# modelscope/dash-infer

Hardware: NVIDIA H100
Metric: decode tokens/sec/GPU Qwen2-7B int4-IQ b=1..64; HBM GB/s vs roofline (higher is better)
Workload: dtype bf16 activations x int4 weights (fp32 accumulate), none KV

## Files before the change

dash-infer_b200/csrc/wq_gemm.cu:

```cuda
#include <cstdio>
#include <cstdlib>
#include <cstring>
#include <map>
#include <mutex>
#include <new>

#include "b2_common.cuh"
#include "comm_shared.cuh"
#include "wq_gemm_shared.cuh"

namespace b2 {

constexpr int kWarps = 8;
constexpr int kThreads = kWarps * 32 + 32;
constexpr int kStageBytes = 8192;
static_assert(kBN == kWarps * 16, "one n16 tile per consumer warp");

struct GemmParams {
  const uint8_t* packed;
  const float2* sz;
  const __nv_bfloat16* A;
  int64_t lda;
  __nv_bfloat16* C;
  int64_t ldc;
  const __nv_bfloat16* bias;
  const __nv_bfloat16* residual;
  float* ws;
  unsigned* counters;
  int M, N, K, Np, KT, NG, S;
  int group_tiles;
  int quanta;
  int xt;
  int nst_log2;
  int act;
  float alpha;
  int cluster;
  int norm_self;
  const __nv_bfloat16* norm_gamma;
  float norm_inv_hidden, norm_eps;
  int comm_on;
  CommDev comm;
};

template <int WBITS>
struct WTraits {
  static constexpr int TILE_BYTES = Image<WBITS>::kTileBytes;
  static constexpr int TPS = kStageBytes / TILE_BYTES > 0 ? kStageBytes / TILE_BYTES : 1;
  static constexpr int STAGE_BYTES = TPS * TILE_BYTES;
};

__device__ __forceinline__ void named_bar_sync(int id, int n) { asm volatile("bar.sync %0, %1;" ::"r"(id), "r"(n) : "memory"); }

// ... 598 lines not shown
          v = (n & 1) ? (b >> 4) : (b & 0xF);
        } else if (WBITS == 8) {
          v = static_cast<const uint8_t*>(src)[(int64_t)k * N + n];
        } else {
          v = static_cast<const uint16_t*>(src)[(int64_t)k * N + n];
        }
      }
      word |= (v ^ flip) << (WBITS * ((e >> 1) + (e & 1) * I::kKPerWord / 2));
    }
    dst[i] = I::kRotated ? (word << 3) | (word >> 29) : word;
  }
}

__global__ void pack_sz_kernel(float2* __restrict__ dst, const __nv_bfloat16* __restrict__ scales,
                               const __nv_bfloat16* __restrict__ zeros, const __nv_bfloat16* __restrict__ scales2,
                               const __nv_bfloat16* __restrict__ zeros2, int pair, int G, int N, int Np, float zbias, int fp16) {
  const int64_t total = (int64_t)G * Np;
  for (int64_t i = blockIdx.x * (int64_t)blockDim.x + threadIdx.x; i < total; i += (int64_t)gridDim.x * blockDim.x) {
    const int np = i % Np, gi = i / Np;
    const int r = np & (kBN - 1), ng = np / kBN;
    const int n = pair ? ng * 64 + (r & 63) : np;
    const __nv_bfloat16* sc = (pair && r >= 64) ? scales2 : scales;
    const __nv_bfloat16* zr = (pair && r >= 64) ? zeros2 : zeros;
    float2 v = make_float2(0.f, 0.f);
    if (n < N) {
      const __nv_bfloat16 sv = sc[(int64_t)gi * N + n], zv = zr[(int64_t)gi * N + n];
      v = fp16 ? make_float2(Ft<true>::to_f(sv), Ft<true>::to_f(zv) + zbias) : make_float2(Ft<false>::to_f(sv), Ft<false>::to_f(zv) + zbias);
    }
    dst[i] = v;
  }
}

}

using namespace b2;

struct Plan {
  bool valid = false;
  int S = 1, xt = 1, smem = 0, quanta = 1, nst_log2 = 2;
  bool cluster = false;
};

struct b2_gemm_wq {
  b2_gemm_wq_desc d;
  int Kp = 0, Np = 0, KT = 0, NG = 0, G = 1, group_tiles = 0;
  int group_k = 0;
  size_t packed_bytes = 0;
  void* packed = nullptr;
  bool own_packed = false;
  float2* sz = nullptr;
  bool own_sz = false;
  unsigned* counters = nullptr;
  Plan plans[2];
  int tc_S = 0;
  bool pair = false;
  int device = 0;
};

typedef void (*gemm_kernel_t)(const GemmParams);

static gemm_kernel_t pick_kernel(int wbits, bool grouped, int mt, bool fp16) {
  return with_wbits(wbits, [&](auto W) {
    return with_flag(grouped, [&](auto G) {
      return with_flag(mt == 1, [&](auto MT1) {
        return with_flag(fp16, [&](auto H) { return wq_gemm_kernel<W, MT1 ? 1 : 2, G && W != 16, H>; });
      });
    });
  });
}
static int stage_bytes_of(int wbits) { return with_wbits(wbits, [](auto W) { return WTraits<W>::STAGE_BYTES; }); }

cudaError_t b2::raise_smem_limit(const void* kern, int smem) {
  static std::mutex mu;
  static std::map<const void*, int> limit;
  std::lock_guard<std::mutex> lk(mu);
  int& cur = limit[kern];
  if (smem <= cur) return cudaSuccess;
  cudaError_t e = cudaFuncSetAttribute(kern, cudaFuncAttributeMaxDynamicSharedMemorySize, smem);
  if (e == cudaSuccess) cur = smem;
  return e;
}

static int make_plan(b2_gemm_wq* h, int mti) {
  Plan& pl = h->plans[mti];
  if (pl.valid) return B2_OK;
  const int mt = 1 << mti, MP = 8 * mt;
  const bool grouped = h->group_tiles > 0;
  const int gt = grouped ? h->group_tiles : 1;
  const int quanta = h->KT / gt;
  const int sms = sm_count();
  gemm_kernel_t kern = pick_kernel(h->d.wbits, grouped, mt, h->d.ft == B2_DT_F16);
  const int ring_kb = env_int("B2_GEMM_RING_KB", 32);
  auto log2_stages = [&](int kb) {
    int l = 1;
    while ((2 << l) * stage_bytes_of(h->d.wbits) <= kb * 1024) ++l;
    return l;
  };
  int nst_log2 = log2_stages(ring_kb);
  const int tps = with_wbits(h->d.wbits, [](auto W) { return WTraits<W>::TPS; });
  const int xq = gt > tps ? gt : tps;
  const int x_budget = env_int("B2_GEMM_XBYTES", 20 * 1024);
  int xt_cap = (x_budget / (MP + 1) - 16) / 128;
  xt_cap = xt_cap / xq * xq;
  if (xt_cap < xq) xt_cap = xq;
  auto smem_for = [&](int xt, int nl2) {
    const int gpc = grouped ? xt / gt : 1;
    return (1 << nl2) * stage_bytes_of(h->d.wbits) + (MP + 1) * (xt * 128 + 16) + MP * kBN * 4 + MP * gpc * 4 + 2 * MP * 4 + 16 + 8 +
// ... 141 lines not shown
  if (int st = launch_failed("pack_weights")) return st;
  if (d.wbits != 16) {
    if (!h->sz || !h->own_sz) {
      B2_CUDA_TRY(cudaMalloc(&h->sz, sizeof(float2) * (size_t)h->G * h->Np));
      h->own_sz = true;
    }
    const float b0 = d.ft == B2_DT_F16 ? 128.f : 16.f;
    const float zbias = d.wbits == 4 ? b0 : (d.qtype == B2_DT_I8 ? 17.f * b0 + 128.f : 17.f * b0);
    const int64_t tot = (int64_t)h->G * h->Np;
    pack_sz_kernel<<<(int)((tot + 255) / 256), 256, 0, stream>>>(h->sz, (const __nv_bfloat16*)scales, (const __nv_bfloat16*)zeros,
                                                                 (const __nv_bfloat16*)scales2, (const __nv_bfloat16*)zeros2, pair,
                                                                 h->G, d.N, h->Np, zbias, d.ft == B2_DT_F16 ? 1 : 0);
    if (int st = launch_failed("pack_sz")) return st;
  }
  return B2_OK;
}

int b2_gemm_wq_prepare_weights(b2_gemm_wq_t h, const void* qdata, const void* scales, const void* zeros,
                               void* packed_dst, void* stream_) {
  if (h && h->pair) return B2_ERR_PARAM;
  return prepare_impl(h, qdata, scales, zeros, nullptr, nullptr, nullptr, packed_dst, stream_);
}

int b2_gemm_wq_prepare_swiglu(b2_gemm_wq_t h, const void* q_gate, const void* s_gate, const void* z_gate, const void* q_up,
                              const void* s_up, const void* z_up, void* stream_) {
  if (!h || !h->pair) return B2_ERR_PARAM;
  return prepare_impl(h, q_gate, s_gate, z_gate, q_up, s_up, z_up, nullptr, stream_);
}

int b2_gemm_wq_attach_packed(b2_gemm_wq_t h, const void* packed, const void* scales_f32, const void* zeros_f32) {
  (void)zeros_f32;
  if (!h || !packed) return B2_ERR_PARAM;
  if (h->own_packed && h->packed) cudaFree(h->packed);
  h->packed = const_cast<void*>(packed);
  h->own_packed = false;
  if (scales_f32) {
    if (h->own_sz && h->sz) cudaFree(h->sz);
    h->sz = (float2*)const_cast<void*>(scales_f32);
    h->own_sz = false;
  }
  return B2_OK;
}

static int mt_index_for(int M) { return M <= 8 ? 0 : 1; }

constexpr int kTcMinM = 17;

static bool use_tc(const b2_gemm_wq* h, int M) {
  if (h->group_k > 0) return true;
  return M >= kTcMinM && (h->group_tiles == 0 || h->d.wbits == 4);
}

static void make_tc_plan(b2_gemm_wq* h) {
  if (h->tc_S > 0) return;
  const int ctas = env_int("B2_GEMM_TC_CTAS_PER_SM", 1);
  auto split_for = [&](int slots, int smax) {
    int S = slots / h->NG;
    if (S > h->KT / 4) S = h->KT / 4;
    if (S > smax) S = smax;
    return S < 1 ? 1 : S;
  };
  h->tc_S = split_for(ctas * sm_count(), env_int("B2_GEMM_TC_MAX_SPLIT", 6));
}

static size_t tc_workspace_bytes(b2_gemm_wq* h) {
  make_tc_plan(h);
  return h->tc_S <= 1 ? 16 : (size_t)h->NG * h->tc_S * kTcMaxM * kBN * sizeof(float) + 16;
}

static int run_tc(b2_gemm_wq* h, TcParams p, int M, cudaStream_t stream) {
  make_tc_plan(h);
  if (h->tc_S > 1 && !p.ws) return B2_ERR_PARAM;
  p.packed = (const uint8_t*)h->packed; p.sz = h->sz; p.counters = h->counters;
  p.N = h->d.N; p.K = h->d.K; p.Np = h->Np; p.KT = h->KT; p.NG = h->NG; p.S = h->tc_S;
  const int64_t a_row = p.a_scale ? p.lda : 2 * p.lda;
  for (int m0 = 0; m0 < M; m0 += kTcMaxM) {
    TcParams q = p;
    q.M = (M - m0) > kTcMaxM ? kTcMaxM : (M - m0);
    q.A = reinterpret_cast<const __nv_bfloat16*>(reinterpret_cast<const uint8_t*>(p.A) + m0 * a_row);
    q.C = p.C + (int64_t)m0 * p.ldc;
    if (p.residual) q.residual = p.residual + (int64_t)m0 * p.ldc;
    if (p.a_scale) {
      q.a_scale = p.a_scale + m0;
      q.tile_sums = p.tile_sums + (size_t)m0 * p.KT;
    }
    if (p.norm_sumsq) q.norm_sumsq = p.norm_sumsq + m0;
    if (p.xg_out) {
      q.sumsq_out = p.sumsq_out + m0;
      q.xg_out = p.xg_out + (int64_t)m0 * p.ldxg;
    }
    cudaError_t e = tc_launch(h->d.wbits, h->d.ft == B2_DT_F16, q, stream);
    if (e != cudaSuccess) {
      set_last_error(p.a_scale ? "wq_gemm_tc (fp8) launch" : "wq_gemm_tc launch", e);
      return B2_ERR_CUDA;
    }
  }
  return B2_OK;
}

size_t b2_gemm_wq_workspace_bytes(b2_gemm_wq_t h, int M) {
  if (!h || M <= 0) return 0;
  if (use_tc(h, M)) return tc_workspace_bytes(h);
  const int mc = M > kGemvMaxM ? kGemvMaxM : M;
  const int mti = mt_index_for(mc);
  if (make_plan(h, mti) != B2_OK) return 0;
  const Plan& pl = h->plans[mti];
  if (pl.S <= 1 || pl.cluster) return 16;
  return (size_t)h->NG * pl.S * (8 << mti) * (kBN + 1) * sizeof(float) + 16;
}

size_t b2_gemm_wq_algo_bytes(b2_gemm_wq_t h, int M) {
  if (!h) return 0;
  const b2_gemm_wq_desc& d = h->d;
  const size_t mul = h->pair ? 2 : 1;
  size_t w = mul * (size_t)d.K * d.N * d.wbits / 8;
  size_t prm = d.wbits == 16 ? 0 : mul * (size_t)2 * 2 * h->G * d.N;
  return w + prm + (size_t)2 * M * ((size_t)d.K + d.N);
}

int b2_gemm_wq_sumsq_parts(b2_gemm_wq_t h) { return h ? h->NG : 0; }

int b2_gemm_wq_run(b2_gemm_wq_t h, const void* A, int64_t lda, void* C, int64_t ldc, int M, const void* bias,
                   const void* residual, int activation, float alpha, void* workspace, size_t workspace_bytes,
                   void* stream_) {
  return b2_gemm_wq_run_fused(h, A, lda, C, ldc, M, bias, residual, activation, alpha, workspace, workspace_bytes, nullptr, stream_);
}

// ... 172 lines not shown
```

dash-infer_b200/csrc/wq_gemm_shared.cuh:

```cuda
#pragma once
#include <cuda.h>

#include <type_traits>

#include "b2_common.cuh"

namespace b2 {

constexpr int kBN = 128;
constexpr int kBK = 64;
constexpr uint32_t kMask4 = 0x00780078u;
constexpr uint32_t kMagic = 0x41804180u;
constexpr uint32_t kMagicHi = 0x43804380u;

template <int WBITS>
struct Image {
  static constexpr int kChunks = WBITS == 4 ? 2 : (WBITS == 8 ? 4 : 8);
  static constexpr int kKPerChunk = kBK / kChunks;
  static constexpr int kKPerWord = kKPerChunk / 4;
  static constexpr int kChunkBytes = kBN * 16;
  static constexpr int kTileBytes = kChunks * kChunkBytes;
  static constexpr int kTileWords = kTileBytes / 4;
  static constexpr bool kRotated = WBITS != 16;
  __host__ __device__ __forceinline__ static int swz(int c) {
    return WBITS == 4 ? 4 * (c & 1) : (WBITS == 8 ? 2 * (c & 3) : 2 * ((c >> 1) & 3));
  }
  __host__ __device__ __forceinline__ static int row_offset(int row, int c) { return (row ^ swz(c)) << 4; }
  __host__ __device__ __forceinline__ static int chunk_offset(const int& row, int c) { return c * kChunkBytes + ((row ^ swz(c)) << 4); }
};

template <typename F>
inline auto with_wbits(int wbits, F&& f) {
  if (wbits == 4) return f(std::integral_constant<int, 4>{});
  if (wbits == 8) return f(std::integral_constant<int, 8>{});
  return f(std::integral_constant<int, 16>{});
}

struct TcParams {
  const uint8_t* packed;
  const float2* sz;
  const __nv_bfloat16* A;
  int64_t lda;
  __nv_bfloat16* C;
  int64_t ldc;
  const __nv_bfloat16* bias;
  const __nv_bfloat16* residual;
  float* ws;
  unsigned* counters;
  int M, N, K, Np, KT, NG, S;
  int act;
  float alpha;
  const float* a_scale = nullptr;
  const float* tile_sums = nullptr;
  const float* norm_sumsq = nullptr;
  int norm_parts = 0, norm_ld = 0;
  float norm_inv_hidden = 0.f, norm_eps = 0.f;
  float* sumsq_out = nullptr;
  __nv_bfloat16* xg_out = nullptr;
  const __nv_bfloat16* gamma_out = nullptr;
  int64_t ldxg = 0;
  int nm;
  int group_tiles = 0;
  int group_k = 0, ngroups = 1;
};

struct Gemv2Params {
  const uint8_t* packed;
  const __nv_bfloat16* A;
  int64_t lda;
  __nv_bfloat16* C;
  int64_t ldc;
  const __nv_bfloat16* bias;
  const __nv_bfloat16* residual;
  int M, N, K, KT, NG;
  int cb_log2;
  int xt;
  int nst_log2;
  int pair;
  int act;
  float alpha;
};
struct Gemv2Plan {
  int mt, grid, smem;
};
bool gemv2_plan(Gemv2Params& p, Gemv2Plan* plan);
cudaError_t gemv2_launch(const Gemv2Params& p, const Gemv2Plan& plan, cudaStream_t stream);

constexpr int kGemvMaxM = 16;
constexpr int kTcMaxM = 64;
cudaError_t tc_launch(int wbits, bool fp16, TcParams p, cudaStream_t stream);

cudaError_t raise_smem_limit(const void* kern, int smem);

typedef CUresult (*EncodeTiledFn)(CUtensorMap*, CUtensorMapDataType, cuuint32_t, void*, const cuuint64_t*, const cuuint64_t*,
                                  const cuuint32_t*, const cuuint32_t*, CUtensorMapInterleave, CUtensorMapSwizzle,
                                  CUtensorMapL2promotion, CUtensorMapFloatOOBfill);
EncodeTiledFn encode_tiled();

}
```

dash-infer_b200/csrc/wq_gemm_tc.cu:

```cuda
#include <type_traits>

#include "b2_common.cuh"
#include "wq_gemm_shared.cuh"

namespace b2 {

constexpr int kTcThreads = 384;
constexpr int kTcNM = 64;
constexpr int kTcNSW = 6;
constexpr int kTcNSX = 3;
constexpr int kTcXTile = kTcNM * 128;

__device__ __forceinline__ void wg_fence() { asm volatile("wgmma.fence.sync.aligned;" ::: "memory"); }
__device__ __forceinline__ void wg_commit() { asm volatile("wgmma.commit_group.sync.aligned;" ::: "memory"); }
template <int N>
__device__ __forceinline__ void wg_wait() { asm volatile("wgmma.wait_group.sync.aligned %0;" ::"n"(N) : "memory"); }
__device__ __forceinline__ void wg_fence_acc(float (&d)[32]) {
#pragma unroll
  for (int i = 0; i < 32; ++i) asm volatile("" : "+f"(d[i])::"memory");
}
__device__ __forceinline__ uint64_t wg_desc(uint32_t saddr) {
  return (uint64_t)((saddr >> 4) & 0x3FFF) | ((uint64_t)1 << 16) | ((uint64_t)(1024 >> 4) << 32) | ((uint64_t)1 << 62);
}

// ... 39 lines not shown
}

__device__ __forceinline__ uint32_t tc_prmt(uint32_t a, uint32_t b, uint32_t sel) {
  uint32_t d;
  asm("prmt.b32 %0, %1, %2, %3;" : "=r"(d) : "r"(a), "r"(b), "r"(sel));
  return d;
}
__device__ __forceinline__ uint32_t lds32(uint32_t addr) {
  uint32_t v;
  asm volatile("ld.shared.u32 %0, [%1];" : "=r"(v) : "r"(addr));
  return v;
}
__device__ __forceinline__ uint32_t nib4_to_e4m3(uint32_t w_rot3, uint32_t qsh, uint32_t msel) {
  const uint32_t word = __funnelshift_r(w_rot3, w_rot3, 3);
  const uint32_t sel = (word & 0x77777777u) >> qsh;
  const uint32_t T0 = 0x44403800u, T1 = 0x4E4C4A48u, H0 = 0x53525150u, H1 = 0x57565554u;
  const uint32_t lo = tc_prmt(T0, T1, sel), hi = tc_prmt(H0, H1, sel);
  const uint32_t m = tc_prmt(word << 4, word, msel);
  uint32_t r;
  asm("lop3.b32 %0, %1, %2, %3, 0xD8;" : "=r"(r) : "r"(lo), "r"(hi), "r"(m));
  return r;
}

template <int WBITS, bool MULTI, bool A8 = false, bool GROUPED = false, bool H = false>
__global__ void __launch_bounds__(kTcThreads, 1) wq_gemm_tc_kernel(const TcParams p, const __grid_constant__ CUtensorMap amap) {
  using I = Image<WBITS>;
  constexpr int TILE_BYTES = I::kTileBytes;
  constexpr int NSW = WBITS == 16 ? 4 : kTcNSW;
  constexpr int TPS = WBITS == 4 ? 4 : 2;
  constexpr int KIND = A8 ? 2 : (H ? 1 : 0);
  static_assert(!A8 || WBITS == 4, "fp8 activations: int4 weights only");
  static_assert(!H || !A8, "fp8 activations come with bf16 outputs");
  using F = Ft<H>;
  static_assert(!GROUPED || (!A8 && WBITS != 16), "sub-channel weights: bf16 activations, int4 / int8");
  const int XTILE_LD = p.nm * 128;
  constexpr int XTPS = A8 ? TPS / 2 : TPS;
  constexpr int WSTAGE = TPS * TILE_BYTES;
  constexpr int XSTAGE = XTPS * kTcXTile;
  extern __shared__ uint8_t smem_raw[];
  uint8_t* smem = reinterpret_cast<uint8_t*>((reinterpret_cast<uintptr_t>(smem_raw) + 1023) & ~uintptr_t(1023));
  uint8_t* xring = smem;
  uint8_t* wring = xring + kTcNSX * XSTAGE;
  float* suma = reinterpret_cast<float*>(wring + NSW * WSTAGE);
  uint64_t* bars = reinterpret_cast<uint64_t*>(suma + kTcNM);
  uint64_t* wfull = bars;
  uint64_t* wfree = wfull + kTcNSW;
  uint64_t* afull = wfree + kTcNSW;
  uint64_t* xsum = afull + kTcNSX;
  uint64_t* xfree = xsum + kTcNSX;
  float* ascale = reinterpret_cast<float*>(bars) + 64;
  __shared__ int s_is_last;

  const int tid = threadIdx.x, warp = tid >> 5, lane = tid & 31;
  const int nunits = p.NG * p.S;

  if (tid == 0) {
    for (int i = 0; i < NSW; ++i) { mbar_init(&wfull[i], 1); mbar_init(&wfree[i], 8); }
    for (int i = 0; i < kTcNSX; ++i) { mbar_init(&afull[i], 1); mbar_init(&xsum[i], 2); mbar_init(&xfree[i], 8); }
    fence_mbar_init();
  }
  __syncthreads();
  pdl_launch_dependents();

  int w_pre = 0;
  const int my_units = !MULTI ? 1 : ((int)blockIdx.x < nunits) ? (nunits - (int)blockIdx.x + (int)gridDim.x - 1) / (int)gridDim.x : 0;
  auto body = [&](auto n32) {
  constexpr bool N32 = decltype(n32)::value;
  for (int uit = 0; uit < my_units; ++uit) {
  const int unit = (int)blockIdx.x + uit * (int)gridDim.x;
  const int ng = unit / p.S;
  const int s = unit - ng * p.S;
  const int kt0 = (int)((int64_t)s * p.KT / p.S), kt1 = (int)((int64_t)(s + 1) * p.KT / p.S);
  const int nt = kt1 - kt0;
  const int nst = (nt + TPS - 1) / TPS;
  const int gbase = MULTI ? uit * nst : 0;
  if (warp == 8) {
    if (lane == 0) {
      auto issue = [&](int g, const uint8_t* src, uint32_t bytes) {
        const int slot = g % NSW;
        if (g >= NSW) mbar_wait_backoff(&wfree[slot], ((g / NSW) & 1) ^ 1);
        mbar_arrive_expect_tx(&wfull[slot], bytes);
        bulk_g2s(wring + slot * WSTAGE, src, bytes, &wfull[slot]);
      };
      const uint8_t* wsrc = p.packed + ((size_t)ng * p.KT + kt0) * TILE_BYTES;
      for (int st = w_pre; st < nst; ++st) issue(gbase + st, wsrc + (size_t)st * WSTAGE, min(TPS, nt - st * TPS) * TILE_BYTES);
      w_pre = 0;
      const int nu = unit + gridDim.x;
      if (MULTI && nu < nunits) {
        const int ng2 = nu / p.S, s2 = nu - ng2 * p.S;
        const int k0 = (int)((int64_t)s2 * p.KT / p.S), k1 = (int)((int64_t)(s2 + 1) * p.KT / p.S);
        const int nt2 = k1 - k0, nst2 = (nt2 + TPS - 1) / TPS;
        const uint8_t* wsrc2 = p.packed + ((size_t)ng2 * p.KT + k0) * TILE_BYTES;
        w_pre = min(NSW, nst2);
        for (int st = 0; st < w_pre; ++st)
          issue(gbase + nst + st, wsrc2 + (size_t)st * WSTAGE, min(TPS, nt2 - st * TPS) * TILE_BYTES);
      }
    }
  } else if (warp == 9) {
    if (lane == 0) {
      pdl_wait();
      for (int st = 0; st < nst; ++st) {
        const int g = gbase + st;
        const int slot = g % kTcNSX;
        if (g >= kTcNSX) {
          const uint32_t par = ((g / kTcNSX) & 1) ^ 1;
          mbar_wait_backoff(&xfree[slot], par);
          mbar_wait_backoff(&xsum[slot], par);
        }
        const int wtiles = min(TPS, nt - st * TPS);
        const int tiles = A8 ? (wtiles + 1) / 2 : wtiles;
        mbar_arrive_expect_tx(&afull[slot], tiles * XTILE_LD);
        for (int ti = 0; ti < tiles; ++ti)
          asm volatile("cp.async.bulk.tensor.2d.shared::cluster.global.mbarrier::complete_tx::bytes [%0], [%1, {%2, %3}], [%4];"
                       ::"r"(smem_u32(xring + slot * XSTAGE + ti * kTcXTile)), "l"(reinterpret_cast<uint64_t>(&amap)),
                         "r"((kt0 + st * TPS + (A8 ? 2 * ti : ti)) * kBK), "r"(0), "r"(smem_u32(&afull[slot]))
                       : "memory");
      }
    }
  } else if (warp >= 10) {
    const int xt = tid - 320;
    float r0 = 0.f, r1 = 0.f, r2 = 0.f, r3 = 0.f;
    if (A8) {
      pdl_wait();
      if (xt < p.M) {
        const float* ts = p.tile_sums + (size_t)xt * p.KT;
        for (int kt = kt0; kt < kt1; ++kt) r0 += ts[kt];
        ascale[xt] = p.a_scale[xt];
      } else {
        ascale[xt] = 0.f;
      }
    }
    if (!A8 && p.norm_sumsq) {
      pdl_wait();
      float ss = 0.f;
      if (xt < p.M)
        for (int i = 0; i < p.norm_parts; ++i) ss += __ldcg(p.norm_sumsq + (size_t)i * p.norm_ld + xt);
      ascale[xt] = rsqrtf(ss * p.norm_inv_hidden + p.norm_eps);
    }
    for (int st = 0; st < nst; ++st) {
      const int g = gbase + st;
      const int slot = g % kTcNSX;
      mbar_wait(&afull[slot], (g / kTcNSX) & 1);
      const int tiles = (WBITS == 16 || A8 || GROUPED || xt >= p.nm) ? 0 : min(TPS, nt - st * TPS);
      for (int ti = 0; ti < tiles; ++ti) {
        const uint32_t rbase = smem_u32(xring + slot * XSTAGE + ti * kTcXTile) + xt * 128;
#pragma unroll
        for (int c = 0; c < 8; c += 2) {
          const uint4 v = lds128(rbase + ((c ^ (xt & 7)) << 4));
          const uint4 w = lds128(rbase + (((c + 1) ^ (xt & 7)) << 4));
          r0 += (F::lo(v.x) + F::hi(v.x)) + (F::lo(v.y) + F::hi(v.y));
          r1 += (F::lo(v.z) + F::hi(v.z)) + (F::lo(v.w) + F::hi(v.w));
          r2 += (F::lo(w.x) + F::hi(w.x)) + (F::lo(w.y) + F::hi(w.y));
          r3 += (F::lo(w.z) + F::hi(w.z)) + (F::lo(w.w) + F::hi(w.w));
        }
      }
      __syncwarp();
      if (lane == 0) mbar_arrive(&xsum[slot]);
    }
    suma[xt] = (r0 + r1) + (r2 + r3);
    asm volatile("bar.sync 3, 320;" ::: "memory");
  } else {
    const int wg = warp >> 2, g8 = lane >> 2, t4 = lane & 3;
    const int rr0 = wg * 64 + (warp & 3) * 16 + g8, rr1 = rr0 + 8;
    const float2 sz0 = (WBITS == 16 || GROUPED) ? make_float2(1.f, 0.f) : p.sz[ng * kBN + rr0];
    const float2 sz1 = (WBITS == 16 || GROUPED) ? make_float2(1.f, 0.f) : p.sz[ng * kBN + rr1];
    const uint32_t wring_u = smem_u32(wring), xring_u = smem_u32(xring);
    uint32_t off0[I::kChunks], off1[I::kChunks];
#pragma unroll
    for (int c = 0; c < I::kChunks; ++c) {
      off0[c] = I::chunk_offset(rr0, c);
      off1[c] = I::chunk_offset(rr1, c);
    }
    const uint32_t sh4 = 4 * t4, sh8 = 8 * (t4 & 1), qsh = 16 * (t4 & 1), msel = (t4 & 1) ? 0xFBEAu : 0xD9C8u;
    const int wa = t4 >> 1;
    auto word = [](const uint4& v, int j) { return j == 0 ? v.x : (j == 1 ? v.y : (j == 2 ? v.z : v.w)); };

    float d[32], dt[32];
#pragma unroll
    for (int i = 0; i < 32; ++i) d[i] = dt[i] = 0.f;
    int prev_xs = -1;
    for (int st = 0; st < nst; ++st) {
      const int g = gbase + st;
      const int slot = g % NSW, xs = g % kTcNSX;
      uint32_t gs2[TPS][2], gc2[TPS][2];
      if (GROUPED && p.group_k == 0) {
#pragma unroll
        for (int ti = 0; ti < TPS; ++ti) {
          const int kt = min(kt0 + st * TPS + ti, kt1 - 1);
          const float2 z0 = __ldg(p.sz + (size_t)(kt / p.group_tiles) * p.Np + ng * kBN + rr0);
          const float2 z1 = __ldg(p.sz + (size_t)(kt / p.group_tiles) * p.Np + ng * kBN + rr1);
          const float c0 = (F::kBias + 8.f - z0.y) * z0.x, c1 = (F::kBias + 8.f - z1.y) * z1.x;
          gs2[ti][0] = F::pack(z0.x, z0.x); gs2[ti][1] = F::pack(z1.x, z1.x);
          gc2[ti][0] = F::pack(c0, c0); gc2[ti][1] = F::pack(c1, c1);
        }
      }
      mbar_wait(&wfull[slot], (g / NSW) & 1);
      mbar_wait(&afull[xs], (g / kTcNSX) & 1);
      const int tiles = min(TPS, nt - st * TPS);
#pragma unroll
      for (int ti = 0; ti < TPS; ++ti) {
        if (ti < tiles) {
          const uint32_t wt = wring_u + slot * WSTAGE + ti * TILE_BYTES;
          if (A8) {
            const uint64_t bd = wg_desc(xring_u + xs * XSTAGE + (ti >> 1) * kTcXTile) + (uint64_t)(4 * (ti & 1));
            uint32_t a[2][4];
#pragma unroll
            for (int c = 0; c < 2; ++c) {
              const uint4 v0 = lds128(wt + off0[c]), v1 = lds128(wt + off1[c]);
              a[c][0] = nib4_to_e4m3(word(v0, wa), qsh, msel);
              a[c][1] = nib4_to_e4m3(word(v1, wa), qsh, msel);
              a[c][2] = nib4_to_e4m3(word(v0, 2 + wa), qsh, msel);
              a[c][3] = nib4_to_e4m3(word(v1, 2 + wa), qsh, msel);
            }
            wg_fence();
#pragma unroll
            for (int c = 0; c < 2; ++c) wg_mma<KIND, N32>(dt, a[c], bd + (uint64_t)(2 * c));
          } else {
            const uint64_t bd = wg_desc(xring_u + xs * XSTAGE + ti * kTcXTile);
            if (WBITS == 4) {
              uint32_t a[4][4];
#pragma unroll
              for (int c = 0; c < 2; ++c) {
                const uint4 v0 = lds128(wt + off0[c]), v1 = lds128(wt + off1[c]);
#pragma unroll
                for (int h = 0; h < 2; ++h) {
                  uint32_t* f = a[2 * c + h];
                  f[0] = lop3_and_or(__funnelshift_r(word(v0, 2 * h), word(v0, 2 * h), sh4), kMask4, F::kMagic);
                  f[1] = lop3_and_or(__funnelshift_r(word(v1, 2 * h), word(v1, 2 * h), sh4), kMask4, F::kMagic);
                  f[2] = lop3_and_or(__funnelshift_r(word(v0, 2 * h + 1), word(v0, 2 * h + 1), sh4), kMask4, F::kMagic);
                  f[3] = lop3_and_or(__funnelshift_r(word(v1, 2 * h + 1), word(v1, 2 * h + 1), sh4), kMask4, F::kMagic);
                  if (GROUPED) {
                    uint32_t sw[4], cw[4];
// ... 35 lines not shown
                a[kk][1] = lds32(wt + off1[2 * kk] + 4 * t4);
                a[kk][2] = lds32(wt + off0[2 * kk + 1] + 4 * t4);
                a[kk][3] = lds32(wt + off1[2 * kk + 1] + 4 * t4);
              }
              wg_fence();
#pragma unroll
              for (int kk = 0; kk < 4; ++kk) wg_mma<KIND, N32>(d, a[kk], bd + (uint64_t)(2 * kk));
            } else {
              uint32_t lo[4][4], hi[4][4];
#pragma unroll
              for (int c = 0; c < 4; ++c) {
                const uint4 v0 = lds128(wt + off0[c]), v1 = lds128(wt + off1[c]);
                const uint32_t w[4] = {word(v0, wa), word(v1, wa), word(v0, 2 + wa), word(v1, 2 + wa)};
#pragma unroll
                for (int e = 0; e < 4; ++e) {
                  lo[c][e] = lop3_and_or(__funnelshift_r(w[e], w[e], sh8), kMask4, F::kMagic);
                  hi[c][e] = lop3_and_or(__funnelshift_r(w[e], w[e], sh8 + 4), kMask4, F::kMagicHi);
                }
              }
              wg_fence();
#pragma unroll
              for (int c = 0; c < 4; ++c) {
                wg_mma<KIND, N32>(d, lo[c], bd + (uint64_t)(2 * c));
                wg_mma<KIND, N32>(d, hi[c], bd + (uint64_t)(2 * c));
              }
            }
          }
          wg_commit();
          wg_wait<1>();
          if (ti == 0 && prev_xs >= 0) {
            __syncwarp();
            if (lane == 0) mbar_arrive(&xfree[prev_xs]);
            prev_xs = -1;
          }
          if (A8 && ((ti & 1) || ti + 1 == tiles)) {
            wg_wait<0>();
            wg_fence_acc(dt);
#pragma unroll
            for (int i = 0; i < 32; ++i) { d[i] += dt[i]; dt[i] = 0.f; }
          }
        }
      }
      __syncwarp();
      if (lane == 0) mbar_arrive(&wfree[slot]);
      prev_xs = xs;
    }
    wg_wait<0>();
    wg_fence_acc(d);
    __syncwarp();
    if (prev_xs >= 0 && lane == 0) mbar_arrive(&xfree[prev_xs]);

    asm volatile("bar.sync 3, 320;" ::: "memory");
    float* fs = reinterpret_cast<float*>(xring);
#pragma unroll
    for (int j = 0; j < 8; ++j) {
      const int m = 8 * j + 2 * t4;
      float s0 = 1.f, s1 = 1.f;
      if (A8 || p.norm_sumsq) { s0 = ascale[m]; s1 = ascale[m + 1]; }
      const float zz0 = A8 ? sz0.y - 16.f : sz0.y, zz1 = A8 ? sz1.y - 16.f : sz1.y;
      const float sa0 = suma[m], sa1 = suma[m + 1];
      fs[m * kBN + rr0] = sz0.x * s0 * (d[4 * j + 0] - zz0 * sa0);
      fs[(m + 1) * kBN + rr0] = sz0.x * s1 * (d[4 * j + 1] - zz0 * sa1);
      fs[m * kBN + rr1] = sz1.x * s0 * (d[4 * j + 2] - zz1 * sa0);
      fs[(m + 1) * kBN + rr1] = sz1.x * s1 * (d[4 * j + 3] - zz1 * sa1);
    }
  }

  pdl_wait();
  __syncthreads();
  {
    constexpr int T = kTcThreads;
    const float4* fs4 = reinterpret_cast<const float4*>(xring);
    float4* fs4w = reinterpret_cast<float4*>(xring);
    const int units = p.M * (kBN / 4);
    constexpr int MPK4 = kTcNM * kBN / 4;
    bool finalize = true;
    if (p.S > 1) {
      float4* wsu = reinterpret_cast<float4*>(p.ws) + ((size_t)ng * p.S + s) * MPK4;
      for (int i = tid; i < units; i += T) wsu[i] = fs4[i];
      __threadfence();
      __syncthreads();
      if (tid == 0) {
        const unsigned prev = atomicAdd(&p.counters[ng], 1u);
        s_is_last = (prev == (unsigned)(p.S - 1));
      }
      __syncthreads();
      finalize = s_is_last != 0;
      if (finalize) {
        __threadfence();
        const float4* wsg = reinterpret_cast<const float4*>(p.ws) + (size_t)ng * p.S * MPK4;
        for (int i0 = tid; i0 < units; i0 += 2 * T) {
          float4 a[2];
          a[0] = a[1] = make_float4(0.f, 0.f, 0.f, 0.f);
          for (int s0 = 0; s0 < p.S; s0 += 8) {
            float4 b[2][8];
#pragma unroll
            for (int g = 0; g < 2; ++g)
#pragma unroll
              for (int u = 0; u < 8; ++u) {
                const int i = i0 + g * T;
                b[g][u] = (s0 + u < p.S && i < units) ? __ldcg(wsg + (size_t)(s0 + u) * MPK4 + i) : make_float4(0.f, 0.f, 0.f, 0.f);
              }
#pragma unroll
            for (int g = 0; g < 2; ++g)
#pragma unroll
              for (int u = 0; u < 8; ++u) { a[g].x += b[g][u].x; a[g].y += b[g][u].y; a[g].z += b[g][u].z; a[g].w += b[g][u].w; }
          }
#pragma unroll
          for (int g = 0; g < 2; ++g) {
            const int i = i0 + g * T;
            if (i < units) fs4w[i] = a[g];
          }
        }
        if (tid == 0) p.counters[ng] = 0;
        __syncthreads();
      }
    }
    if (finalize) {
      const bool vec_ok = (p.ldc & 3) == 0 && (reinterpret_cast<uintptr_t>(p.C) & 7) == 0;
      if (p.act == B2_ACT_SWIGLU) {
        const int su = p.M * 16;
#pragma unroll 1
        for (int i = tid; i < su; i += T) {
          const int m = i >> 4, nq = i & 15;
          const int nn = ng * 64 + nq * 4;
          if (nn >= p.N) continue;
          const float4 gv = fs4[m * 32 + nq], uv = fs4[m * 32 + 16 + nq];
          float v[4];
          v[0] = apply_act<B2_ACT_SILU>(gv.x * p.alpha) * (uv.x * p.alpha);
          v[1] = apply_act<B2_ACT_SILU>(gv.y * p.alpha) * (uv.y * p.alpha);
          v[2] = apply_act<B2_ACT_SILU>(gv.z * p.alpha) * (uv.z * p.alpha);
          v[3] = apply_act<B2_ACT_SILU>(gv.w * p.alpha) * (uv.w * p.alpha);
          __nv_bfloat16* cp = p.C + (int64_t)m * p.ldc + nn;
          if (vec_ok && nn + 3 < p.N) {
            *reinterpret_cast<uint2*>(cp) = make_uint2(F::pack(v[0], v[1]), F::pack(v[2], v[3]));
          } else {
#pragma unroll
            for (int e = 0; e < 4; ++e)
              if (nn + e < p.N) cp[e] = F::from_f(v[e]);
          }
        }
      } else if (p.act == B2_ACT_NONE && vec_ok && (p.N & 3) == 0 &&
                 (!p.residual || (reinterpret_cast<uintptr_t>(p.residual) & 7) == 0) &&
                 (!p.bias || (reinterpret_cast<uintptr_t>(p.bias) & 7) == 0)) {
        constexpr int UPT = (kTcNM * (kBN / 4) + T - 1) / T;
        uint2 res[UPT];
#pragma unroll
        for (int j = 0; j < UPT; ++j) {
          const int i = tid + j * T;
          const int m = i >> 5, nn = ng * kBN + (i & 31) * 4;
          res[j] = make_uint2(0u, 0u);
          if (p.residual && i < units && nn < p.N) res[j] = __ldg(reinterpret_cast<const uint2*>(p.residual + (int64_t)m * p.ldc + nn));
        }
#pragma unroll
// ... 7 lines not shown
            if (p.bias) {
              const uint2 bv = __ldg(reinterpret_cast<const uint2*>(p.bias + nn));
              v0 += F::lo(bv.x); v1 += F::hi(bv.x); v2 += F::lo(bv.y); v3 += F::hi(bv.y);
            }
            v0 += F::lo(res[j].x); v1 += F::hi(res[j].x); v2 += F::lo(res[j].y); v3 += F::hi(res[j].y);
            const uint2 st2 = make_uint2(F::pack(v0, v1), F::pack(v2, v3));
            *reinterpret_cast<uint2*>(p.C + (int64_t)m * p.ldc + nn) = st2;
            if (p.xg_out) {
              const float r0 = F::lo(st2.x), r1 = F::hi(st2.x), r2 = F::lo(st2.y), r3 = F::hi(st2.y);
              const uint2 gv = __ldg(reinterpret_cast<const uint2*>(p.gamma_out + nn));
              *reinterpret_cast<uint2*>(p.xg_out + (int64_t)m * p.ldxg + nn) =
                  make_uint2(F::pack(r0 * F::lo(gv.x), r1 * F::hi(gv.x)), F::pack(r2 * F::lo(gv.y), r3 * F::hi(gv.y)));
              ssq = (r0 * r0 + r1 * r1) + (r2 * r2 + r3 * r3);
            }
          }
          if (p.xg_out) {
#pragma unroll
            for (int o = 16; o > 0; o >>= 1) ssq += __shfl_xor_sync(0xffffffffu, ssq, o);
            if (lane == 0 && i < units) p.sumsq_out[(size_t)ng * p.norm_ld + m] = ssq;
          }
        }
      } else {
        const float* fs = reinterpret_cast<const float*>(xring);
#pragma unroll 1
        for (int i = tid; i < p.M * (kBN / 2); i += T) {
          const int m = i >> 6, np = i & 63;
          const int nn = ng * kBN + np * 2;
          if (nn >= p.N) continue;
          float v0 = fs[m * kBN + np * 2] * p.alpha, v1 = fs[m * kBN + np * 2 + 1] * p.alpha;
          const bool has1 = (nn + 1) < p.N;
          if (p.bias) {
            v0 += F::to_f(p.bias[nn]);
            if (has1) v1 += F::to_f(p.bias[nn + 1]);
          }
          v0 = apply_act_rt(v0, p.act);
          v1 = apply_act_rt(v1, p.act);
          __nv_bfloat16* cp = p.C + (int64_t)m * p.ldc + nn;
          if (p.residual) {
            const __nv_bfloat16* rp = p.residual + (int64_t)m * p.ldc + nn;
            v0 += F::to_f(rp[0]);
            if (has1) v1 += F::to_f(rp[1]);
          }
          if (has1 && ((reinterpret_cast<uintptr_t>(cp) & 3) == 0)) {
            *reinterpret_cast<uint32_t*>(cp) = F::pack(v0, v1);
          } else {
            cp[0] = F::from_f(v0);
            if (has1) cp[1] = F::from_f(v1);
          }
        }
      }
    }
  }

  if (MULTI) asm volatile("fence.proxy.async.shared::cta;" ::: "memory");
  __syncthreads();
  }
  };
  if (p.nm == 32)
    body(std::true_type{});
  else
    body(std::false_type{});
}

template <int WBITS>
static int tc_smem_bytes() {
  const int tps = WBITS == 4 ? 4 : 2;
  const int wstage = tps * Image<WBITS>::kTileBytes;
  const int nsw = WBITS == 16 ? 4 : kTcNSW;
  return 1024 + kTcNSX * tps * kTcXTile + nsw * wstage + kTcNM * 4 + 96 * 8 + 64;
}

EncodeTiledFn encode_tiled() {
  static EncodeTiledFn fn = nullptr;
  if (!fn) {
    void* p = nullptr;
    cudaDriverEntryPointQueryResult q;
    if (cudaGetDriverEntryPoint("cuTensorMapEncodeTiled", &p, cudaEnableDefault, &q) == cudaSuccess && q == cudaDriverEntryPointSuccess)
      fn = reinterpret_cast<EncodeTiledFn>(p);
  }
  return fn;
}

cudaError_t tc_launch(int wbits, bool fp16, TcParams p, cudaStream_t stream) {
  EncodeTiledFn enc = encode_tiled();
  if (!enc) return cudaErrorNotSupported;
  alignas(64) CUtensorMap amap;
  const bool a8 = p.a_scale != nullptr;
  const cuuint64_t gdim[2] = {(cuuint64_t)p.K, (cuuint64_t)p.M};
  const cuuint64_t gstride[1] = {(cuuint64_t)p.lda * (a8 ? 1 : 2)};
  static const int n32 = env_int("B2_GEMM_TC_N32", 1);
  p.nm = (n32 && p.M <= 32) ? 32 : kTcNM;
  const cuuint32_t box[2] = {(cuuint32_t)(a8 ? 2 * kBK : kBK), (cuuint32_t)p.nm};
  const cuuint32_t estr[2] = {1, 1};
  if (enc(&amap, a8 ? CU_TENSOR_MAP_DATA_TYPE_UINT8 : CU_TENSOR_MAP_DATA_TYPE_BFLOAT16, 2, const_cast<__nv_bfloat16*>(p.A), gdim, gstride, box, estr,
          CU_TENSOR_MAP_INTERLEAVE_NONE, CU_TENSOR_MAP_SWIZZLE_128B, CU_TENSOR_MAP_L2_PROMOTION_L2_128B,
          CU_TENSOR_MAP_FLOAT_OOB_FILL_NONE) != CUDA_SUCCESS)
    return cudaErrorInvalidValue;

  static const int persist = env_int("B2_GEMM_TC_PERSIST", 1);
  const int units = p.NG * p.S;
  const int cap = sm_count();
  const int grid = (persist && units > cap) ? cap : units;
  const bool grouped = p.group_tiles > 0 || p.group_k > 0;
  if ((a8 && (wbits != 4 || fp16)) || (grouped && !a8 && wbits != 4)) return cudaErrorNotSupported;
  return with_wbits(wbits, [&](auto W) {
    const size_t smem = (size_t)tc_smem_bytes<W>();
    auto go = [&](auto kern) {
      const cudaError_t e = raise_smem_limit((const void*)kern, (int)smem);
      return e != cudaSuccess ? e : launch(kern, dim3(grid), dim3(kTcThreads), smem, stream, true, p, amap);
    };
    return with_flag(units > grid, [&](auto MULTI) {
      if constexpr (W == 4) {
        if (a8) return go(wq_gemm_tc_kernel<4, MULTI, true>);
      }
      return with_flag(grouped, [&](auto G) {
        return with_flag(fp16, [&](auto H) { return go(wq_gemm_tc_kernel<W, MULTI, false, G && W == 4, H>); });
      });
    });
  });
}

}
```

Baseline: 8739.

## Balance persistent TC GEMM tail wave by splitting remainder tiles across two CTAs

Replaces the uniform split-K/persistent scheduler with a segment schedule. When the number of N-groups exceeds the SM count, the leftover tail groups are split in half along K. One CTA computes the first half and writes its raw accumulators and activation sums to a carry buffer. A second, otherwise idle CTA continues from that carry, or recomputes the whole K range if the carry is not yet ready. This targets the idle SMs in the last wave for large-N layers, at the cost of extra workspace, atomics and possible redundant work when the carry arrives late.

```diff
diff --git a/dash-infer_b200/csrc/wq_gemm.cu b/dash-infer_b200/csrc/wq_gemm.cu
--- a/dash-infer_b200/csrc/wq_gemm.cu
+++ b/dash-infer_b200/csrc/wq_gemm.cu
@@ -1,3 +1,4 @@
+#include <algorithm>
 #include <cstdio>
 #include <cstdlib>
 #include <cstring>
@@ -702,7 +703,7 @@
   bool own_sz = false;
   unsigned* counters = nullptr;
   Plan plans[2];
-  int tc_S = 0;
+  int tc_grid = 0, tc_rounds = 0, tc_S = 1, tc_h = 0;
   bool pair = false;
   int device = 0;
 };
@@ -950,27 +951,36 @@
 }
 
 static void make_tc_plan(b2_gemm_wq* h) {
-  if (h->tc_S > 0) return;
-  const int ctas = env_int("B2_GEMM_TC_CTAS_PER_SM", 1);
-  auto split_for = [&](int slots, int smax) {
-    int S = slots / h->NG;
-    if (S > h->KT / 4) S = h->KT / 4;
-    if (S > smax) S = smax;
-    return S < 1 ? 1 : S;
-  };
-  h->tc_S = split_for(ctas * sm_count(), env_int("B2_GEMM_TC_MAX_SPLIT", 6));
+  if (h->tc_grid > 0) return;
+  const int sms = sm_count(), NG = h->NG, KT = h->KT;
+  const int smax = std::max(1, env_int("B2_GEMM_TC_MAX_SPLIT", 6));
+  if (NG <= sms || !env_int("B2_GEMM_TC_PERSIST", 1)) {
+    h->tc_S = std::max(1, std::min({sms / NG, KT / 4, smax}));
+    h->tc_grid = NG * h->tc_S;
+    h->tc_rounds = 0;
+    h->tc_h = 0;
+    return;
+  }
+  const int NR = NG % sms;
+  h->tc_S = 1;
+  h->tc_grid = sms;
+  h->tc_rounds = NG / sms;
+  h->tc_h = (NR > 0 && smax > 1 && 2 * NR <= sms) ? KT / 2 / 4 * 4 : 0;
 }
 
 static size_t tc_workspace_bytes(b2_gemm_wq* h) {
   make_tc_plan(h);
-  return h->tc_S <= 1 ? 16 : (size_t)h->NG * h->tc_S * kTcMaxM * kBN * sizeof(float) + 16;
+  if (h->tc_S > 1) return (size_t)h->NG * h->tc_S * kTcMaxM * kBN * sizeof(float) + 16;
+  if (h->tc_h > 0) return (size_t)(h->NG - h->tc_rounds * h->tc_grid) * kTcCarryFloats * sizeof(float) + 16;
+  return 16;
 }
 
 static int run_tc(b2_gemm_wq* h, TcParams p, int M, cudaStream_t stream) {
   make_tc_plan(h);
-  if (h->tc_S > 1 && !p.ws) return B2_ERR_PARAM;
+  if ((h->tc_S > 1 || h->tc_h > 0) && !p.ws) return B2_ERR_PARAM;
   p.packed = (const uint8_t*)h->packed; p.sz = h->sz; p.counters = h->counters;
-  p.N = h->d.N; p.K = h->d.K; p.Np = h->Np; p.KT = h->KT; p.NG = h->NG; p.S = h->tc_S;
+  p.N = h->d.N; p.K = h->d.K; p.Np = h->Np; p.KT = h->KT; p.NG = h->NG;
+  p.grid = h->tc_grid; p.rounds = h->tc_rounds; p.S = h->tc_S; p.h = h->tc_h;
   const int64_t a_row = p.a_scale ? p.lda : 2 * p.lda;
   for (int m0 = 0; m0 < M; m0 += kTcMaxM) {
     TcParams q = p;
diff --git a/dash-infer_b200/csrc/wq_gemm_shared.cuh b/dash-infer_b200/csrc/wq_gemm_shared.cuh
--- a/dash-infer_b200/csrc/wq_gemm_shared.cuh
+++ b/dash-infer_b200/csrc/wq_gemm_shared.cuh
@@ -47,7 +47,8 @@
   const __nv_bfloat16* residual;
   float* ws;
   unsigned* counters;
-  int M, N, K, Np, KT, NG, S;
+  int M, N, K, Np, KT, NG;
+  int grid, rounds, S, h;
   int act;
   float alpha;
   const float* a_scale = nullptr;
@@ -62,6 +63,32 @@
   int nm;
   int group_tiles = 0;
   int group_k = 0, ngroups = 1;
+};
+
+struct TcSeg {
+  int ng, kt0, kt1;
+  int part, parts;
+  int carry;
+};
+constexpr int kTcCarryFloats = 256 * 32 + 64 * 4;
+struct TcSched {
+  int NG, KT, grid, rounds, S, h, b, nfull, NR;
+  __host__ __device__ TcSched(int NG_, int KT_, int grid_, int rounds_, int S_, int h_, int b_)
+      : NG(NG_), KT(KT_), grid(grid_), rounds(rounds_), S(S_), h(h_), b(b_), nfull(rounds_ * grid_), NR(NG_ - rounds_ * grid_) {}
+  __host__ __device__ int count() const {
+    return rounds == 0 ? 1 : rounds + (b < NR ? 1 : 0) + (h > 0 && b >= NR && b < 2 * NR ? 1 : 0);
+  }
+  __host__ __device__ TcSeg seg(int i) const {
+    if (rounds == 0) {
+      const int ng = b / S, s = b - ng * S;
+      return TcSeg{ng, s * KT / S, (s + 1) * KT / S, s, S, 0};
+    }
+    const int head = b < NR ? 1 : 0;
+    if (head && i == 0) return TcSeg{nfull + b, 0, h > 0 ? h : KT, 0, 1, h > 0 ? 1 : 0};
+    const int j = i - head;
+    if (j < rounds) return TcSeg{j * grid + b, 0, KT, 0, 1, 0};
+    return TcSeg{nfull + b - NR, h, KT, 0, 1, 2};
+  }
 };
 
 struct Gemv2Params {
diff --git a/dash-infer_b200/csrc/wq_gemm_tc.cu b/dash-infer_b200/csrc/wq_gemm_tc.cu
--- a/dash-infer_b200/csrc/wq_gemm_tc.cu
+++ b/dash-infer_b200/csrc/wq_gemm_tc.cu
@@ -115,7 +115,10 @@
   __shared__ int s_is_last;
 
   const int tid = threadIdx.x, warp = tid >> 5, lane = tid & 31;
-  const int nunits = p.NG * p.S;
+  const TcSched sch(p.NG, p.KT, (int)gridDim.x, p.rounds, p.S, p.h, (int)blockIdx.x);
+  const int nseg = MULTI ? sch.count() : 1;
+  auto segment = [&](int i) { return sch.seg(i); };
+  __shared__ unsigned s_carry;
 
   if (tid == 0) {
     for (int i = 0; i < NSW; ++i) { mbar_init(&wfull[i], 1); mbar_init(&wfree[i], 8); }
@@ -126,17 +129,27 @@
   pdl_launch_dependents();
 
   int w_pre = 0;
-  const int my_units = !MULTI ? 1 : ((int)blockIdx.x < nunits) ? (nunits - (int)blockIdx.x + (int)gridDim.x - 1) / (int)gridDim.x : 0;
   auto body = [&](auto n32) {
   constexpr bool N32 = decltype(n32)::value;
-  for (int uit = 0; uit < my_units; ++uit) {
-  const int unit = (int)blockIdx.x + uit * (int)gridDim.x;
-  const int ng = unit / p.S;
-  const int s = unit - ng * p.S;
-  const int kt0 = (int)((int64_t)s * p.KT / p.S), kt1 = (int)((int64_t)(s + 1) * p.KT / p.S);
+  int gbase = 0;
+  for (int si = 0; si < nseg; ++si) {
+  const TcSeg sg = segment(si);
+  const int ng = sg.ng, kt1 = sg.kt1;
+  bool carry_in = false;
+  if (MULTI && sg.carry == 2) {
+    pdl_wait();
+    if (tid == 0) {
+      s_carry = atomicAdd(&p.counters[ng], 1u);
+      if (s_carry == 1u) p.counters[ng] = 0;
+      __threadfence();
+    }
+    __syncthreads();
+    carry_in = s_carry == 1u;
+  }
+  const int kt0 = sg.carry == 2 && !carry_in ? 0 : sg.kt0;
+  const float* carry_src = p.ws + (size_t)(ng - sch.nfull) * kTcCarryFloats;
   const int nt = kt1 - kt0;
   const int nst = (nt + TPS - 1) / TPS;
-  const int gbase = MULTI ? uit * nst : 0;
   if (warp == 8) {
     if (lane == 0) {
       auto issue = [&](int g, const uint8_t* src, uint32_t bytes) {
@@ -148,12 +161,10 @@
       const uint8_t* wsrc = p.packed + ((size_t)ng * p.KT + kt0) * TILE_BYTES;
       for (int st = w_pre; st < nst; ++st) issue(gbase + st, wsrc + (size_t)st * WSTAGE, min(TPS, nt - st * TPS) * TILE_BYTES);
       w_pre = 0;
-      const int nu = unit + gridDim.x;
-      if (MULTI && nu < nunits) {
-        const int ng2 = nu / p.S, s2 = nu - ng2 * p.S;
-        const int k0 = (int)((int64_t)s2 * p.KT / p.S), k1 = (int)((int64_t)(s2 + 1) * p.KT / p.S);
-        const int nt2 = k1 - k0, nst2 = (nt2 + TPS - 1) / TPS;
-        const uint8_t* wsrc2 = p.packed + ((size_t)ng2 * p.KT + k0) * TILE_BYTES;
+      if (si + 1 < nseg && segment(si + 1).carry != 2) {
+        const TcSeg s2 = segment(si + 1);
+        const int nt2 = s2.kt1 - s2.kt0, nst2 = (nt2 + TPS - 1) / TPS;
+        const uint8_t* wsrc2 = p.packed + ((size_t)s2.ng * p.KT + s2.kt0) * TILE_BYTES;
         w_pre = min(NSW, nst2);
         for (int st = 0; st < w_pre; ++st)
           issue(gbase + nst + st, wsrc2 + (size_t)st * WSTAGE, min(TPS, nt2 - st * TPS) * TILE_BYTES);
@@ -183,6 +194,10 @@
   } else if (warp >= 10) {
     const int xt = tid - 320;
     float r0 = 0.f, r1 = 0.f, r2 = 0.f, r3 = 0.f;
+    if (carry_in) {
+      const float4 r = __ldcg(reinterpret_cast<const float4*>(carry_src + 256 * 32) + xt);
+      r0 = r.x; r1 = r.y; r2 = r.z; r3 = r.w;
+    }
     if (A8) {
       pdl_wait();
       if (xt < p.M) {
@@ -222,6 +237,8 @@
     }
     suma[xt] = (r0 + r1) + (r2 + r3);
     asm volatile("bar.sync 3, 320;" ::: "memory");
+    if (MULTI && sg.carry == 1)
+      reinterpret_cast<float4*>(xring)[256 * 32 / 4 + xt] = make_float4(r0, r1, r2, r3);
   } else {
     const int wg = warp >> 2, g8 = lane >> 2, t4 = lane & 3;
     const int rr0 = wg * 64 + (warp & 3) * 16 + g8, rr1 = rr0 + 8;
@@ -241,6 +258,13 @@
     float d[32], dt[32];
 #pragma unroll
     for (int i = 0; i < 32; ++i) d[i] = dt[i] = 0.f;
+    if (carry_in) {
+#pragma unroll
+      for (int i = 0; i < 32; i += 4) {
+        const float4 v = __ldcg(reinterpret_cast<const float4*>(carry_src + tid * 32 + i));
+        d[i] = v.x; d[i + 1] = v.y; d[i + 2] = v.z; d[i + 3] = v.w;
+      }
+    }
     int prev_xs = -1;
     for (int st = 0; st < nst; ++st) {
       const int g = gbase + st;
@@ -382,6 +406,11 @@
 
     asm volatile("bar.sync 3, 320;" ::: "memory");
     float* fs = reinterpret_cast<float*>(xring);
+    if (MULTI && sg.carry == 1) {
+#pragma unroll
+      for (int i = 0; i < 32; i += 4)
+        reinterpret_cast<float4*>(fs + tid * 32)[i / 4] = make_float4(d[i], d[i + 1], d[i + 2], d[i + 3]);
+    } else {
 #pragma unroll
     for (int j = 0; j < 8; ++j) {
       const int m = 8 * j + 2 * t4;
@@ -394,6 +423,7 @@
       fs[m * kBN + rr1] = sz1.x * s0 * (d[4 * j + 2] - zz1 * sa0);
       fs[(m + 1) * kBN + rr1] = sz1.x * s1 * (d[4 * j + 3] - zz1 * sa1);
     }
+    }
   }
 
   pdl_wait();
@@ -405,31 +435,39 @@
     const int units = p.M * (kBN / 4);
     constexpr int MPK4 = kTcNM * kBN / 4;
     bool finalize = true;
-    if (p.S > 1) {
-      float4* wsu = reinterpret_cast<float4*>(p.ws) + ((size_t)ng * p.S + s) * MPK4;
+    if (MULTI && sg.carry == 1) {
+      float4* dst = reinterpret_cast<float4*>(p.ws + (size_t)(ng - sch.nfull) * kTcCarryFloats);
+      for (int i = tid; i < kTcCarryFloats / 4; i += T) dst[i] = fs4[i];
+      __threadfence();
+      __syncthreads();
+      if (tid == 0 && atomicAdd(&p.counters[ng], 1u) == 1u) p.counters[ng] = 0;
+      finalize = false;
+    } else if (sg.parts > 1) {
+      const size_t slots = (size_t)ng * p.S;
+      float4* wsu = reinterpret_cast<float4*>(p.ws) + (slots + sg.part) * MPK4;
       for (int i = tid; i < units; i += T) wsu[i] = fs4[i];
       __threadfence();
       __syncthreads();
       if (tid == 0) {
         const unsigned prev = atomicAdd(&p.counters[ng], 1u);
-        s_is_last = (prev == (unsigned)(p.S - 1));
+        s_is_last = (prev == (unsigned)(sg.parts - 1));
       }
       __syncthreads();
       finalize = s_is_last != 0;
       if (finalize) {
         __threadfence();
-        const float4* wsg = reinterpret_cast<const float4*>(p.ws) + (size_t)ng * p.S * MPK4;
+        const float4* wsg = reinterpret_cast<const float4*>(p.ws) + slots * MPK4;
         for (int i0 = tid; i0 < units; i0 += 2 * T) {
           float4 a[2];
           a[0] = a[1] = make_float4(0.f, 0.f, 0.f, 0.f);
-          for (int s0 = 0; s0 < p.S; s0 += 8) {
+          for (int s0 = 0; s0 < sg.parts; s0 += 8) {
             float4 b[2][8];
 #pragma unroll
             for (int g = 0; g < 2; ++g)
 #pragma unroll
               for (int u = 0; u < 8; ++u) {
                 const int i = i0 + g * T;
-                b[g][u] = (s0 + u < p.S && i < units) ? __ldcg(wsg + (size_t)(s0 + u) * MPK4 + i) : make_float4(0.f, 0.f, 0.f, 0.f);
+                b[g][u] = (s0 + u < sg.parts && i < units) ? __ldcg(wsg + (size_t)(s0 + u) * MPK4 + i) : make_float4(0.f, 0.f, 0.f, 0.f);
               }
 #pragma unroll
             for (int g = 0; g < 2; ++g)
@@ -543,8 +581,9 @@
     }
   }
 
-  if (MULTI) asm volatile("fence.proxy.async.shared::cta;" ::: "memory");
+  asm volatile("fence.proxy.async.shared::cta;" ::: "memory");
   __syncthreads();
+  gbase += nst;
   }
   };
   if (p.nm == 32)
@@ -588,10 +627,7 @@
           CU_TENSOR_MAP_FLOAT_OOB_FILL_NONE) != CUDA_SUCCESS)
     return cudaErrorInvalidValue;
 
-  static const int persist = env_int("B2_GEMM_TC_PERSIST", 1);
-  const int units = p.NG * p.S;
-  const int cap = sm_count();
-  const int grid = (persist && units > cap) ? cap : units;
+  const int grid = p.grid;
   const bool grouped = p.group_tiles > 0 || p.group_k > 0;
   if ((a8 && (wbits != 4 || fp16)) || (grouped && !a8 && wbits != 4)) return cudaErrorNotSupported;
   return with_wbits(wbits, [&](auto W) {
@@ -600,7 +636,7 @@
       const cudaError_t e = raise_smem_limit((const void*)kern, (int)smem);
       return e != cudaSuccess ? e : launch(kern, dim3(grid), dim3(kTcThreads), smem, stream, true, p, amap);
     };
-    return with_flag(units > grid, [&](auto MULTI) {
+    return with_flag(p.NG > grid, [&](auto MULTI) {
       if constexpr (W == 4) {
         if (a8) return go(wq_gemm_tc_kernel<4, MULTI, true>);
       }
```

Measured after the change: 9054, median of 6. 3.6% higher.
